# ag14774/OpenCL-Lattice-Boltzmann

Hardware: AMD Instinct MI355X
Metric: MLUPS (higher is better)
Workload: dtype f32

## Files before the change

opencl-lattice-boltzmann_amd/csrc/core_interval.h:

```cpp
#pragma once

#if defined(__HIPCC__) || defined(__CUDACC__)
#define LBM_CORE_HD __host__ __device__ inline
#else
#define LBM_CORE_HD inline
#endif

namespace lbm {

struct CoreInterval {
  int kc0, kc1;
};

LBM_CORE_HD CoreInterval core_interval(int ys, int ye, int L, int ny, bool up, bool twinned, int accel_row, int accel_row_b,
                                       bool accel_next) {
  const int n = ye - ys, d = up ? 1 : -1;
  const int lead = twinned ? 0 : L - 1, sf = twinned ? 1 : 2;
  const int r0 = up ? ys - lead : ye - 1 + lead;
  const CoreInterval none = {0, 0};
  if (n <= 0 || L < 2) return none;
  int lo = lead + L - 1, hi = n + lead - 1;
  const int k_steady = sf * (L - 1) + 1;
  if (lo < k_steady) lo = k_steady;
  if (up) {
// ... 3 lines not shown
    if (lo < kmin) lo = kmin;
  } else {
    const int kmax = (r0 - 1) - 1;
    if (hi > kmax) hi = kmax;
    const int kmin = r0 - (ny - 2) - 1;
    if (lo < kmin) lo = kmin;
  }
  if (hi - lo + 1 < 2) return none;
  const int Lacc = accel_next ? L : L - 1;
  int c0[2], c1[2], nc = 0;
  const int arows[2] = {accel_row, accel_row_b};
  for (int i = 0; i < 2; i++) {
    const int A = arows[i];
    if (A < 0 || A >= ny || Lacc <= 0) continue;
    const int kA = (A - r0) * d;
    if (kA + Lacc - 1 < lo || kA > hi) continue;
    int j = nc++;
    if (j == 1 && kA < c0[0]) { c0[1] = c0[0]; c1[1] = c1[0]; j = 0; }
    c0[j] = kA;
    c1[j] = kA + Lacc - 1;
  }
  int best0 = 0, best1 = 0;
  int start = lo;
  for (int i = 0; i <= nc; i++) {
    const int end = i < nc ? c0[i] : hi + 1;
    if (end - start > best1 - best0) { best0 = start; best1 = end; }
    if (i < nc && c1[i] + 1 > start) start = c1[i] + 1;
  }
  if (best1 - best0 < 2) return none;
  const CoreInterval r = {best0, best1};
  return r;
}

}
```

opencl-lattice-boltzmann_amd/csrc/d2q9_kernels.h:

```cpp
#pragma once
#include <type_traits>

#include <hip/hip_runtime.h>
#include <stdint.h>

#include "core_interval.h"

namespace lbm {

constexpr int kBlock = 256;

struct StepArgs {
  const float *src;
  float *dst;
  const uint8_t *mask;
  const float *south_src[3];
  const float *north_src[3];
  float *partials;
  unsigned long long plane_stride;
  unsigned long long row_stride;
  int nx, rows;
  int y_begin, y_count;
  int y_split, y_begin2;
  int accel_row;
  float omega, aw1, aw2;
};


__device__ __forceinline__ float wave_sum(float v) {
  for (int o = 32; o > 0; o >>= 1) v += __shfl_xor(v, o, 64);
  return v;
}

__device__ __forceinline__ double wave_sum(double v) {
  for (int o = 32; o > 0; o >>= 1) v += __shfl_xor(v, o, 64);
  return v;
}

typedef float v4f __attribute__((ext_vector_type(4)));
// ... 1418 lines not shown
    in.h0 = lo ? Rc[1 * ps + xhalo_w] : Rc[3 * ps + xhalo_e];
    in.h1 = lo ? Rs[5 * ps + xhalo_w] : Rs[6 * ps + xhalo_e];
    in.h2 = lo ? Rn[8 * ps + xhalo_w] : Rn[7 * ps + xhalo_e];
  }
}

typedef __attribute__((address_space(1))) v2f global_v2f;
constexpr int kPairSlotFloats = 128;
constexpr int kPairWinFloats = 9 * kPairSlotFloats;
struct PairWindow { v2f mid[3], S0[3], S1[3]; };
struct __attribute__((packed, aligned(4))) f2u { float x, y; };
__device__ __forceinline__ v2f lds_pair(const float *p) { return *reinterpret_cast<const v2f *>(p); }
__device__ __forceinline__ v2f lds_pair_shifted(const float *p) {
  const f2u t = *reinterpret_cast<const f2u *>(p);
  v2f r = {t.x, t.y};
  return r;
}
__device__ __forceinline__ void lds_pair_put(float *p, v2f v) { *reinterpret_cast<v2f *>(p) = v; }

__device__ __forceinline__ void issue_pair_loads_at(const float *Rc, size_t ps, size_t rs, int xcol, PairLoads &in) {
  unsigned xb = (unsigned)xcol * 4u;
  asm volatile("" : "+v"(xb));
  auto ld = [&](const float *p) {
    unsigned long long pk = (unsigned long long)p;
    asm volatile("" : "+s"(pk));
    return *(const global_v2f *)(pk + xb);
  };
  const float *const Rs = Rc - rs, *const Rn = Rc + rs;
  in.c[0] = ld(Rc); in.c[1] = ld(Rc + ps); in.c[3] = ld(Rc + 3 * ps);
  in.c[2] = ld(Rs + 2 * ps); in.c[5] = ld(Rs + 5 * ps); in.c[6] = ld(Rs + 6 * ps);
  in.c[4] = ld(Rn + 4 * ps); in.c[7] = ld(Rn + 7 * ps); in.c[8] = ld(Rn + 8 * ps);
}

constexpr int deep_halo_lanes(int D) { return D / 2; }
constexpr bool deep_edge_loads(int D) { return 2 * deep_halo_lanes(D) < D; }
constexpr int deep_lds_windows(int D) { return D - 1 < 4 ? D - 1 : 4; }

__device__ __forceinline__ bool strip_rows_clean(const unsigned long long *bits, int words, int strip, int lo, int hi, int ny) {
  if (bits == nullptr || hi - lo >= ny) return false;
  const unsigned long long *w = bits + (size_t)strip * words;
  unsigned long long any = 0;
  auto range = [&](int r0, int r1) {
    for (int i = r0 >> 6; i <= (r1 - 1) >> 6; i++) {
      const int b0 = r0 - 64 * i > 0 ? r0 - 64 * i : 0, b1 = r1 - 64 * i < 64 ? r1 - 64 * i : 64;
      const unsigned long long upto = b1 == 64 ? ~0ull : ((1ull << b1) - 1ull);
      any |= w[i] & upto & ~((1ull << b0) - 1ull);
    }
  };
  int l0 = lo % ny;
  if (l0 < 0) l0 += ny;
  const int l1 = l0 + (hi - lo);
  if (l1 <= ny) range(l0, l1);
  else { range(l0, ny); range(0, l1 - ny); }
  return __builtin_amdgcn_readfirstlane((int)(any == 0ull)) != 0;
}
__device__ __forceinline__ void deep_sweep_rows(bool up, bool twinned, int L, int ys, int ye, int *lo, int *hi) {
  const int lead = twinned ? 0 : L - 1, count = (ye - ys) + lead + (L - 1);
  const int first = up ? ys - lead : ye - 1 + lead - (count - 1);
  *lo = first;
  *hi = first + count;
}

static __global__ __launch_bounds__(64) void strip_row_bits(const uint8_t *mask, int nx, int rows, int strips, int lanes_out, int halo_lanes,
                                                     unsigned long long *bits, int words) {
  const int strip = blockIdx.x % strips, word = blockIdx.x / strips, lane = threadIdx.x;
  if (word >= words) return;
  const int q2 = nx >> 1;
  int qw = (strip * lanes_out + lane - halo_lanes) % q2;
  if (qw < 0) qw += q2;
  const int xcol = qw * 2;
  unsigned long long out = 0;
  for (int b = 0; b < 64; b++) {
    const int r = word * 64 + b;
    if (r >= rows) break;
    const uint32_t m = *reinterpret_cast<const uint32_t *>(mask + (size_t)r * nx + (xcol & ~3)) >> ((xcol & 2) * 8);
    if (__builtin_amdgcn_ballot_w64((m & 0xffffu) != 0) != 0ull) out |= 1ull << b;
  }
  if (lane == 0) bits[(size_t)strip * words + word] = out;
}

template <int D, int WL, bool UP, bool NT, bool OBST_PATHS, bool TWIN = false, int LT = 0, bool FREE = false>
__device__ __forceinline__ void deep_sweep(const Step2Args &a, const int L_arg, float *lds, float *partials, int pstride, int ys, int ye,
                                           int xcol, int xhalo_w, int xhalo_e, int lane, bool owner, int unit,
                                           const bool twinned_in = false, float *lds_twin = nullptr) {
  static_assert(LT >= 0 && LT <= D, "steady depth");
  const int L = LT > 0 ? LT : L_arg;
  const bool twinned = TWIN && twinned_in;
  const size_t ps = a.plane_stride;
  auto wrap = [&](int r) { return r < 0 ? r + a.ny : (r >= a.ny ? r - a.ny : r); };
  const int n = ye - ys, d = UP ? 1 : -1;
  const int lead = twinned ? 0 : L - 1;
  const int sf = twinned ? 1 : 2;
  const int r0 = UP ? ys - lead : ye - 1 + lead;
  const int last = n + lead + (L - 1) - 1;
  float sum[D];
  constexpr int NR = (D - 1 - WL) > 0 ? (D - 1 - WL) : 1;
  PairWindow w[NR];
  uint32_t m_mid[D - 1];
#pragma unroll
  for (int l = 0; l < D; l++) sum[l] = 0.f;
#pragma unroll
  for (int l = 0; l < D - 1; l++) m_mid[l] = 0;
#pragma unroll
  for (int l = 0; l < NR; l++) {
#pragma unroll
    for (int i = 0; i < 3; i++) w[l].mid[i] = w[l].S0[i] = w[l].S1[i] = splat2(0.f);
  }
  float *const lw = lds + 2 + 2 * lane;
  uint32_t accbits = 0, ownbits = 0;
  const uint32_t accmask = a.accel_next ? 0xffffffffu : ~(1u << (L - 1));
  const uint32_t mask_shift = (xcol & 2) * 8;
  PairLoads in;
  issue_pair_loads<false, deep_edge_loads(D)>(a, wrap(r0), xcol, xhalo_w, xhalo_e, lane, in);
  float *const mailbox = lw + WL * kPairWinFloats;
  auto window_read = [&](int l, int par, int k, v2f (&q)[6]) __attribute__((always_inline)) {
    if ((l - 1) < WL) {
      const float *W = lw + (l - 1) * kPairWinFloats;
// ... 21 lines not shown
#pragma unroll
      for (int kk = 0; kk < 9; kk++) {
        unsigned long long pk = (unsigned long long)(row + kk * ps);
        asm volatile("" : "+s"(pk));
        global_v2f *const q = (global_v2f *)(pk + xb);
        if (NT) __builtin_nontemporal_store(out[kk], q);
        else *q = out[kk];
      }
    }
  };
  auto store_row = [&](int kprev) __attribute__((always_inline)) { store_row_at(a.dst + (size_t)(r0 + (kprev - (L - 1)) * d) * a.row_stride); };
  constexpr bool HAS_CORE = LT > 0 && FREE && !deep_edge_loads(D);
  const float *core_src = a.src;
  float *core_dst = a.dst;
  const long long core_step = UP ? (long long)a.row_stride : -(long long)a.row_stride;
  auto iteration = [&](const int k, auto lt_tag, auto core_tag) __attribute__((always_inline)) {
    constexpr int LS = decltype(lt_tag)::value;
    constexpr bool STEADY = LS > 0;
    constexpr bool CORE = decltype(core_tag)::value;
    static_assert(!CORE || (STEADY && HAS_CORE), "the CORE form is a steady form of the free sweeps");
    const int LL = STEADY ? LS : L;
    const int par = k & 1;
    v2f top[9], pre[2][6];
    uint32_t m_top;
    if (!CORE) {
      const int row0 = wrap(r0 + k * d);
      accbits = ((accbits << 1) | ((row0 == a.accel_row || row0 == a.accel_row_b) ? 1u : 0u)) & accmask;
      ownbits = (ownbits << 1) | ((k >= lead && k <= n + lead - 1) ? 1u : 0u);
    }
    if (STEADY || k >= sf) window_read(1, par, STEADY ? -1 : k, pre[1]);
    {
      v2f g[9];
      g[0] = in.c[0]; g[2] = in.c[2]; g[4] = in.c[4];
      if (deep_edge_loads(D)) {
        g[1] = pair_from_west(in.c[1], in.h0); g[5] = pair_from_west(in.c[5], in.h1); g[8] = pair_from_west(in.c[8], in.h2);
        g[3] = pair_from_east(in.c[3], in.h0); g[6] = pair_from_east(in.c[6], in.h1); g[7] = pair_from_east(in.c[7], in.h2);
      } else {
        g[1] = pair_from_west(in.c[1]); g[5] = pair_from_west(in.c[5]); g[8] = pair_from_west(in.c[8]);
        g[3] = pair_from_east(in.c[3]); g[6] = pair_from_east(in.c[6]); g[7] = pair_from_east(in.c[7]);
      }
      m_top = FREE ? 0u : in.m >> mask_shift;
      v2f t;
      if (FREE || (OBST_PATHS && __builtin_amdgcn_ballot_w64((m_top & 0xffffu) != 0) == 0ull)) t = collide2<false>(g, m_top, a.omega, !CORE && (accbits & 1u) != 0, a.aw1, a.aw2, top);
      else t = collide2<true>(g, m_top, a.omega, (accbits & 1u) != 0, a.aw1, a.aw2, top);
      if ((CORE || (ownbits & 1u)) && owner) sum[0] += t.x + t.y;
      if (CORE) {
        store_row_at(core_dst);
        issue_pair_loads_at(core_src, ps, a.row_stride, xcol, in);
        core_dst += core_step;
        core_src += core_step;
      } else {
        if (STEADY || k - 1 >= sf * (LL - 1)) store_row(k - 1);
        issue_pair_loads<false, deep_edge_loads(D)>(a, wrap(r0 + (k < last ? k + 1 : k) * d), xcol, xhalo_w, xhalo_e, lane, in);
      }
    }
#pragma unroll
    for (int l = 1; l < D; l++) {
      if (STEADY && l >= LS) break;
      if (STEADY) __builtin_amdgcn_sched_barrier(0);
      const bool final = (l == D - 1) || (l == LL - 1);
      if (!STEADY && TWIN && (l - 1) >= WL && twinned && k == l) __syncthreads();
      v2f nxt[9];
      uint32_t m_nxt = 0;
      const bool active = STEADY || k >= sf * l;
      const bool in_lds = (l - 1) < WL;
      float *const W = lw + (l - 1) * kPairWinFloats;
      float *const Wp = W + (3 + 3 * par) * kPairSlotFloats;
      PairWindow &R = w[in_lds ? 0 : (l - 1 - WL)];
      if (active) {
        const v2f (&q)[6] = pre[l & 1];
        if (l + 1 < D && !final && (STEADY || k >= sf * (l + 1))) window_read(l + 1, par, STEADY ? -1 : k, pre[(l + 1) & 1]);
        v2f g[9];
        g[0] = q[0]; g[1] = q[1]; g[3] = q[2];
        if (UP) {
          g[2] = q[3]; g[5] = q[4]; g[6] = q[5];
          g[4] = top[4]; g[8] = pair_from_west(top[8]); g[7] = pair_from_east(top[7]);
        } else {
          g[4] = q[3]; g[8] = q[4]; g[7] = q[5];
          g[2] = top[2]; g[5] = pair_from_west(top[5]); g[6] = pair_from_east(top[6]);
        }
        m_nxt = FREE ? 0u : m_mid[l - 1];
// ... 12 lines not shown
      if (in_lds) {
        lds_pair_put(W, top[0]); lds_pair_put(W + kPairSlotFloats, top[1]); lds_pair_put(W + 2 * kPairSlotFloats, top[3]);
        lds_pair_put(Wp, UP ? top[2] : top[4]);
        lds_pair_put(Wp + kPairSlotFloats, UP ? top[5] : top[8]);
        lds_pair_put(Wp + 2 * kPairSlotFloats, UP ? top[6] : top[7]);
      } else {
        R.mid[0] = top[0]; R.mid[1] = top[1]; R.mid[2] = top[3];
#pragma unroll
        for (int i = 0; i < 3; i++) R.S0[i] = R.S1[i];
        R.S1[0] = UP ? top[2] : top[4]; R.S1[1] = UP ? top[5] : top[8]; R.S1[2] = UP ? top[6] : top[7];
      }
      if (!FREE) m_mid[l - 1] = m_top;
      if (!STEADY && TWIN && twinned && k == l - 1) {
        float *const Wt = lds_twin + 2 + 2 * lane + (in_lds ? (l - 1) * kPairWinFloats + (3 + 3 * (l & 1)) * kPairSlotFloats : WL * kPairWinFloats);
        lds_pair_put(Wt, UP ? top[4] : top[2]);
        lds_pair_put(Wt + kPairSlotFloats, UP ? top[8] : top[5]);
        lds_pair_put(Wt + 2 * kPairSlotFloats, UP ? top[7] : top[6]);
      }
      if (!active || final) break;
      if (l < D - 1) {
#pragma unroll
        for (int kk = 0; kk < 9; kk++) top[kk] = nxt[kk];
        m_top = m_nxt;
      }
    }
    if (!STEADY && TWIN && twinned && k <= L - 2) __syncthreads();
  };
  const int k_steady = sf * (L - 1) + 1;
  int k = 0;
  if (LT > 0) {
    for (; k < k_steady && k <= last; k++) iteration(k, std::integral_constant<int, 0>{}, std::false_type{});
    if constexpr (HAS_CORE) {
      CoreInterval ci = {0, 0};
      if (a.core_loop) ci = core_interval(ys, ye, L, a.ny, UP, twinned, a.accel_row, a.accel_row_b, a.accel_next != 0);
      const int kc0 = __builtin_amdgcn_readfirstlane(ci.kc0), kc1 = __builtin_amdgcn_readfirstlane(ci.kc1);
      bool core_ahead = kc1 > kc0;
      for (;;) {
        const int stop = core_ahead ? kc0 : last + 1;
        for (; k < stop; k++) iteration(k, std::integral_constant<int, LT>{}, std::false_type{});
        if (!core_ahead) break;
        core_ahead = false;
        core_src = a.src + (long long)(r0 + (kc0 + 1) * d) * (long long)a.row_stride;
        core_dst = a.dst + (long long)(r0 + (kc0 - L) * d) * (long long)a.row_stride;
        for (; k < kc1; k++) iteration(k, std::integral_constant<int, LT>{}, std::true_type{});
        ownbits = (1u << L) - 1u;
        accbits = 0;
      }
    } else {
      for (; k <= last; k++) iteration(k, std::integral_constant<int, LT>{}, std::false_type{});
    }
  } else {
    for (; k <= last; k++) iteration(k, std::integral_constant<int, 0>{}, std::false_type{});
  }
  store_row(last);
#pragma unroll
  for (int l = 0; l < D; l++) {
    if (l >= L) break;
    const float s = wave_sum(sum[l]);
    if (lane == 0) partials[(size_t)l * pstride + unit] = s;
  }
}

__device__ __forceinline__ void push_chunk_pairs(const Step2Args *la, int ys, int ye, int xcol, bool owner) {
  drain_stores();
  const HaloPeer *pp = uniform_ptr(la->peer);
  const int hi0 = __builtin_amdgcn_readfirstlane(pp->row_hi0);
  const int lo0 = __builtin_amdgcn_readfirstlane(pp->row_lo0);
  const int rows = __builtin_amdgcn_readfirstlane(pp->push_rows);
  const int buf = __builtin_amdgcn_readfirstlane(la->peer_buf) & 1;
  const int side = ys >= hi0 ? 1 : 0;
  const int base = side ? hi0 : lo0;
  if (ys < base || ye > base + rows) {
    if ((threadIdx.x & 63) == 0) atomicOr(pp->wait_err, 2u);
    return;
  }
  const size_t rs = la->row_stride, ps = la->plane_stride;
  const float *own = la->dst + xcol;
// ... 34 lines not shown
  if (slot >= us.units_per_band) return;
  const int unit0 = band * us.units_per_band + slot;
  const int sdiv = (PUSH && us.edge) ? a.strips_edge : a.strips;
  const int chunk = unit0 / sdiv;
  int strip = unit0 - chunk * sdiv;
  const int unit = unit0 + us.partial_off;
  int ys, ye;
  if (a.vmap != nullptr && !(PUSH && us.edge)) {
    const int *e = a.vtab + 2 * ((size_t)a.vmap[2 * strip + 1] * a.nchunks + chunk);
    strip = a.vmap[2 * strip];
    ys = e[0];
    ye = e[1];
  } else {
    ys = us.chunk_start[chunk];
    ye = us.chunk_start[chunk + 1];
  }
  if (ys >= ye || chunk == us.skip) {
    if (lane < nlev) partials[(size_t)lane * pstride + unit] = 0.f;
    if constexpr (PUSH) {
      const Step2Args *la = late_args<Step2Args>();
      if (us.edge && (la->peer_mode & 1)) publish_wave_when_last(la->peer, (unsigned)la->edge_units, la->seq);
    }
    return;
  }
  const int q2 = a.nx >> 1;
  const int qcol = strip * a.lanes_out + lane - HL;
  const bool owner = (lane >= HL) && (lane < HL + a.lanes_out) && (qcol < q2);
  int qw = qcol % q2;
  if (qw < 0) qw += q2;
  const int xcol = qw * 2;
  const int xhalo_w = (xcol == 0) ? a.nx - 1 : xcol - 1;
  const int xhalo_e = (xcol + 2 >= a.nx) ? 0 : xcol + 2;
  const bool up = __builtin_amdgcn_readfirstlane((int)((chunk & 1) == 0)) != 0;
  bool clean = false;
  if constexpr (LT > 0 && OBST_PATHS) {
    int lo, hi;
    deep_sweep_rows(up, false, LT, ys, ye, &lo, &hi);
    clean = strip_rows_clean(a.clean_bits, a.clean_words, strip, lo, hi, a.ny);
  }
  if (clean) {
    if constexpr (LT > 0 && OBST_PATHS) {
      if (up) deep_sweep<D, WL, true, NT, OBST_PATHS, false, LT, true>(a, nlev, lds, partials, pstride, ys, ye, xcol, xhalo_w, xhalo_e, lane, owner, unit);
      else deep_sweep<D, WL, false, NT, OBST_PATHS, false, LT, true>(a, nlev, lds, partials, pstride, ys, ye, xcol, xhalo_w, xhalo_e, lane, owner, unit);
    }
  } else if (up) {
    deep_sweep<D, WL, true, NT, OBST_PATHS, false, LT>(a, nlev, lds, partials, pstride, ys, ye, xcol, xhalo_w, xhalo_e, lane, owner, unit);
  } else {
    deep_sweep<D, WL, false, NT, OBST_PATHS, false, LT>(a, nlev, lds, partials, pstride, ys, ye, xcol, xhalo_w, xhalo_e, lane, owner, unit);
  }
  if constexpr (PUSH) {
    const Step2Args *la = late_args<Step2Args>();
    if (do_push) {
      push_chunk_pairs(la, ys, ye, xcol, owner);
      publish_wave_when_last(la->peer, (unsigned)la->edge_units, la->seq);
    }
  }
}

template <int D, bool NT, bool OBST_PATHS = false, int LT = 0, bool PUSH = false>
__global__ __launch_bounds__(128, 2) void d2q9_deep_twin(const Step2Args a, float *partials, int pstride, int nlev) {
  constexpr int WL = deep_lds_windows(D), HL = deep_halo_lanes(D);
  constexpr int kWaveFloats = WL * kPairWinFloats + (D - 1 > WL ? 3 * kPairSlotFloats : 0) + 4;
  constexpr bool EDGE_PAIRS = PUSH && D <= 5;
  __shared__ float lds[2 * kWaveFloats];
  const int lane = threadIdx.x & 63;
  const int wv = __builtin_amdgcn_readfirstlane((int)(threadIdx.x >> 6));
  const UnitSel us = select_unit<PUSH>(a, a.edge_units / 2);
  const bool do_push = PUSH && us.edge && (a.peer_mode & 1);
  if constexpr (PUSH) {
    if (us.edge && (a.peer_mode & 2)) {
      const Step2Args *la = late_args<Step2Args>();
      const HaloPeer *pp = la->peer;
      if (lane < 2) spin_on_flag(pp->wait_flags + lane, la->wait_seq, pp->wait_err, pp->wait_ticks);
    }
  }
  const int band = us.bid % us.nbands, slot = us.bid / us.nbands;
// ... 7 lines not shown
  const int unit = ((edge_wg && EDGE_PAIRS) ? 2 * pair + wv : chunk) * sdiv + strip + us.partial_off;
  int ys, ye, pys, pye;
  if (a.vmap != nullptr && !edge_wg) {
    const int *e = a.vtab + 2 * ((size_t)a.vmap[2 * strip + 1] * a.nchunks + chunk), *pe = e + (wv ? -2 : 2);
    strip = a.vmap[2 * strip];
    ys = e[0]; ye = e[1];
    pys = pe[0]; pye = pe[1];
  } else {
    ys = us.chunk_start[chunk]; ye = us.chunk_start[chunk + 1];
    pys = us.chunk_start[chunk ^ 1]; pye = us.chunk_start[(chunk ^ 1) + 1];
  }
  const bool empty = ys >= ye || (!(PUSH && us.edge) && chunk == us.skip);
  const bool twinned = !(PUSH && us.edge && !EDGE_PAIRS) && !empty && pys < pye && (chunk ^ 1) != us.skip;
  if constexpr (PUSH && !EDGE_PAIRS) {
    if (us.edge && wv == 0 && lane < nlev) partials[(size_t)lane * pstride + (a.strips_edge + strip + us.partial_off)] = 0.f;
  }
  if (empty) {
    if (lane < nlev) partials[(size_t)lane * pstride + unit] = 0.f;
    if constexpr (PUSH) {
      const Step2Args *la = late_args<Step2Args>();
      if (us.edge && (la->peer_mode & 1)) publish_wave_when_last(la->peer, (unsigned)la->edge_units, la->seq);
    }
    return;
  }
  const int q2 = a.nx >> 1;
  const int qcol = strip * a.lanes_out + lane - HL;
  const bool owner = (lane >= HL) && (lane < HL + a.lanes_out) && (qcol < q2);
  int qw = qcol % q2;
  if (qw < 0) qw += q2;
  const int xcol = qw * 2;
  const int xhalo_w = (xcol == 0) ? a.nx - 1 : xcol - 1;
  const int xhalo_e = (xcol + 2 >= a.nx) ? 0 : xcol + 2;
  float *const mine = lds + wv * kWaveFloats, *const theirs = lds + (wv ^ 1) * kWaveFloats;
  bool clean = false;
  if constexpr (LT > 0 && OBST_PATHS && D == 8) {
    int lo, hi;
    deep_sweep_rows(wv != 0, twinned, LT, ys, ye, &lo, &hi);
    clean = strip_rows_clean(a.clean_bits, a.clean_words, strip, lo, hi, a.ny);
  }
  if (clean) {
    if constexpr (LT > 0 && OBST_PATHS && D == 8) {
      if (wv != 0) deep_sweep<D, WL, true, NT, OBST_PATHS, true, LT, true>(a, nlev, mine, partials, pstride, ys, ye, xcol, xhalo_w, xhalo_e, lane, owner, unit, twinned, theirs);
      else deep_sweep<D, WL, false, NT, OBST_PATHS, true, LT, true>(a, nlev, mine, partials, pstride, ys, ye, xcol, xhalo_w, xhalo_e, lane, owner, unit, twinned, theirs);
    }
  } else if (wv != 0) {
    deep_sweep<D, WL, true, NT, OBST_PATHS, true, LT>(a, nlev, mine, partials, pstride, ys, ye, xcol, xhalo_w, xhalo_e, lane, owner, unit, twinned, theirs);
  } else {
    deep_sweep<D, WL, false, NT, OBST_PATHS, true, LT>(a, nlev, mine, partials, pstride, ys, ye, xcol, xhalo_w, xhalo_e, lane, owner, unit, twinned, theirs);
  }
  if constexpr (PUSH) {
    const Step2Args *la = late_args<Step2Args>();
    if (do_push) {
      push_chunk_pairs(la, ys, ye, xcol, owner);
      publish_wave_when_last(la->peer, (unsigned)la->edge_units, la->seq);
    }
  }
}

struct ResidentArgs {
  const float *src;
  float *dst;
  const uint8_t *mask;
  float *partials;
  unsigned long long plane_stride, row_stride, pstride;
  int nx, ny, nsteps;
  int accel_row;
  int accel_next;
  float omega, aw1, aw2;
  unsigned *words;
  float *xrows;
  unsigned seq_base;
  unsigned *err;
  unsigned long long wait_ticks;
};

__device__ __forceinline__ void resident_store(float *p, v2f v) {
// ... 453 lines not shown
```

opencl-lattice-boltzmann_amd/csrc/lbm_hip.cpp:

```cpp
#include "../../include/lbm.h"
#include "d2q9_kernels.h"
#include "deep_instances.h"
#include "chunk_schedule.h"
#include "halo_exchange.h"
#include "lbm_error.h"

#include <dlfcn.h>
#include <rccl/rccl.h>
#include <unistd.h>

#include <algorithm>
#include <cmath>
#include <cstdarg>
#include <cstdio>
#include <cstdlib>
#include <cstring>
#include <string>
#include <vector>

namespace {

thread_local std::string g_err;

int fail(int code, const char *fmt, ...) {
// ... 263 lines not shown
template <typename T>
int dev_alloc(T **p, size_t count) {
  HIP_TRY(hipMalloc(reinterpret_cast<void **>(p), count * sizeof(T)));
  return LBM_OK;
}

int step_blocks(const lbm_ctx *c, int work_rows) {
  const int vec = c->vec4 ? 4 : 1;
  const long threads = (long)(c->p.nx / vec) * work_rows;
  int nb = div_up(threads, kBlock);
  if (c->grid_blocks > 0) nb = std::min(nb, c->grid_blocks);
  return std::max(1, nb);
}

bool windows_in_lds(const lbm_ctx *c) { return c->windows < 0 ? kStep3LdsDefault : c->windows != 0; }
int step3_load_bufs(const lbm_ctx *c) { return c->load_bufs > 0 ? c->load_bufs : (windows_in_lds(c) ? 1 : 2); }

bool step3_can_pair(const lbm_ctx *c) { return windows_in_lds(c) && step3_load_bufs(c) == 1 && c->pair != 0; }

int step3_sched_waves(const lbm_ctx *c) {
  if (c->sched_waves > 0) return c->sched_waves;
  if (!windows_in_lds(c)) return 1;
  if (step3_can_pair(c)) return 2;
  return (long)c->p.nx * c->rows_min <= 800L * 1024 ? 1 : 2;
}
int step4_sched_waves(const lbm_ctx *c) { return c->sched_waves > 0 ? c->sched_waves : 2; }

int pair_taper(const lbm_ctx *c) { return c->pair_taper >= 0 ? c->pair_taper : kPairTaper32; }

bool fuse_possible(const lbm_ctx *c) {
  if (!c->vec4 || c->p.nx < 256) return false;
  return c->rows_min >= 8;
}
bool deep_possible(const lbm_ctx *c) {
  return fuse_possible(c) && c->rows_min >= 4 * kDeepSteps && (!c->halo_mode || c->halo_depth >= kDeepMin);
}
constexpr long kTwinDeepCells = 3L << 20;
constexpr long kSlabDeepCells = 3L << 20;
constexpr long kSlabTwinCells = 300L * 1024;
constexpr int kOneRoundRows = 160;
constexpr int kMaxHeavyStrips = 4;
bool compact_transport(const lbm_ctx *c) { return c->halo_mode && c->transport_eff == TRANSPORT_PEER && c->compact != 0; }
bool stageable_transport(const lbm_ctx *c) {
  if (!c->halo_mode || c->transport_eff != TRANSPORT_RCCL || c->compact == 0 || c->slabs.empty()) return false;
  for (const Slab &s : c->slabs)
    if (!s.can_wait_value) return false;
  return true;
}
bool slab_twin5(const lbm_ctx *c) {
  if ((long)c->p.nx * c->rows_min <= kSlabTwinCells || (long)c->p.nx * c->rows_min >= kSlabDeepCells) return false;
  const bool transport_ok = compact_transport(c) || (stageable_transport(c) && c->halo_depth == kDeepTwinDefault);
  return transport_ok && (c->halo_depth == kDeepTwinDefault || c->halo_depth == kMultiMaxT) && fuse_possible(c) && c->rows_min >= 4 * kDeepTwinDefault &&
         c->pair != 0 && c->multistep <= 0 && (c->fuse < 0 || c->fuse == kDeepTwinDefault) && c->twin_steps <= 0;
}
int twin_cap(const lbm_ctx *c) {
  if (slab_twin5(c)) return kDeepTwinDefault;
  if (c->twin_steps > 0) return c->twin_steps;
  return (long)c->p.nx * c->rows_min >= kTwinDeepCells ? kDeepTwinSteps : kDeepTwinDefault;
}
bool deep_twin_effective(const lbm_ctx *c) {
  if (c->halo_mode || c->slabs.empty() || !c->slabs[0].f6_twin.paired) return false;
  return c->pair != 0;
}
int fuse_level(const lbm_ctx *c) {
  if (!fuse_possible(c)) return 0;
  if (slab_twin5(c)) return kDeepTwinDefault;
  int lvl;
  if (c->fuse >= 0) {
    lvl = c->fuse == 0 ? 0 : (c->fuse >= 3 ? c->fuse : 2);
  } else {
    const long cells = (long)c->p.nx * c->rows_min;
    lvl = cells >= 1280L * 1024 ? 4 : (cells > 450L * 1024 ? 3 : 2);
    if (deep_possible(c) && (cells >= kSlabDeepCells || (cells > 300L * 1024 && deep_twin_effective(c)))) lvl = kDeepSteps;
  }
  if (lvl > 4 && !(lvl >= kDeepMin && lvl <= kDeepSteps && deep_possible(c))) lvl = 4;
  if (lvl >= kDeepMin && c->halo_mode) lvl = std::min(lvl, c->halo_depth);
  if (lvl == 4 && ((c->halo_mode && c->halo_depth < 4) || !windows_in_lds(c))) lvl = 3;
  if (lvl == 3 && c->halo_mode && c->halo_depth < 3) lvl = 2;
  return lvl;
}

bool resident_effective(const lbm_ctx *c) {
  if (c->halo_mode || c->slabs.size() != 1 || c->slabs[0].res_bands <= 0) return false;
  if (c->resident >= 0) return c->resident > 0;
  return c->fuse < 0 && c->multistep < 0 && (long)c->p.nx * c->p.ny >= 200L * 1024;
}
const void *resident_kernel(int bh) {
  return bh == 2 ? (const void *)d2q9_resident<2> : bh == 4 ? (const void *)d2q9_resident<4> : (const void *)d2q9_resident<6>;
}
int resident_geometry(const lbm_ctx *c, Slab &s) {
  s.res_bh = s.res_w = s.res_bands = 0;
  if (c->halo_mode || c->resident == 0 || c->p.nx % 4 != 0 || c->p.nx < 128 || c->p.nx > 1024) return LBM_OK;
  const int W = div_up(c->p.nx, 128);
  if (set_dev(s)) return LBM_ERR_HIP;
  int bh = 0;
  for (int cand : {2, 4, 6}) {
    if (c->p.ny % cand != 0) continue;
    int per_cu = 0;
// ... 384 lines not shown
      for (int y = 0; y < s.edge_rows; y += ec) tab.push_back(s.row0 + s.rows - s.edge_rows + y);
      tab.push_back(s.row0 + s.rows);
      if (tab.size() % 2 == 0) tab.push_back(s.row0 + s.rows);
      if (set_dev(s)) return LBM_ERR_HIP;
      if (e.chunk_start) HIP_TRY(hipFree(e.chunk_start));
      e.chunk_start = nullptr;
      if (dev_alloc(&e.chunk_start, tab.size())) return LBM_ERR_HIP;
      HIP_TRY(hipMemcpy(e.chunk_start, tab.data(), tab.size() * sizeof(int), hipMemcpyHostToDevice));
      e.nchunks = (int)tab.size() - 1;
      e.skip = n_edge_chunks;
      e.nbands = 1;
      e.units_per_band = e.nchunks * s.strips;
      e.units = e.units_per_band;
      const int i0 = s.row0 + s.edge_rows, i1 = s.row0 + s.rows - s.edge_rows;
      if (i1 > i0) {
        const int rsv = compact_sets(c) ? 4 * n_edge_chunks * s.strips : 2 * n_edge_chunks * s.strips;
        if (int rc = fuse_schedule(s, i0, i1, cmax, cmin, true, s.f_main, 2, rsv)) return rc;
        if (int rc = fuse_schedule_pairs(c, s, i0, i1, c3max, c3min, s.f3_main, step3_sched_waves(c), rsv, step3_can_pair(c))) return rc;
        if (int rc = fuse_schedule_pairs(c, s, i0, i1, c4max, c4min, s.f4_main, step4_sched_waves(c), rsv, windows_in_lds(c))) return rc;
      } else {
        s.f_main.units = s.f3_main.units = s.f4_main.units = 0;
        s.f_main.paired = s.f3_main.paired = s.f4_main.paired = false;
      }
      s.nb_total = std::max(s.nb_total, std::max(s.f_main.units, std::max(s.f3_main.units, s.f4_main.units)) + e.units);
    } else {
      if (int rc = fuse_schedule(s, 0, s.rows, cmax, cmin, true, s.f_main)) return rc;
      s.nb_total = std::max(s.nb_total, s.f_main.units);
      if (int rc = fuse_schedule_pairs(c, s, 0, s.rows, c3max, c3min, s.f3_main, step3_sched_waves(c), 0, step3_can_pair(c))) return rc;
      s.nb_total = std::max(s.nb_total, s.f3_main.units);
      if (int rc = fuse_schedule_pairs(c, s, 0, s.rows, c4max, c4min, s.f4_main, step4_sched_waves(c), 0, windows_in_lds(c))) return rc;
      s.nb_total = std::max(s.nb_total, s.f4_main.units);
    }
    if (int rc = deep_geometry(c, s)) return rc;
  }
  if (int rc = resident_geometry(c, s)) return rc;
  return LBM_OK;
}

bool nt_effective(const lbm_ctx *c) {
  if (c->nt_stores >= 0) return c->nt_stores != 0;
  const size_t grid_bytes = c->slabs[0].row_stride * c->slabs[0].ext_rows * sizeof(float);
  return 2 * grid_bytes > ((size_t)192 << 20);
}

int effective_mode(const lbm_ctx *c) {
  if (!c->vec4) return LM_SCALAR;
  const bool wave_rows = (c->p.nx % 256 == 0);
  int m = c->variant > 0 ? c->variant - 1 : (wave_rows ? LM_DPP : LM_SCALAR);
  if ((m == LM_DPP || m == LM_LDS) && !wave_rows) m = LM_SCALAR;
  return m;
}

enum { KIND_NONE = 0, KIND_SINGLE = 1, KIND_FUSED2 = 2, KIND_MULTI = 3, KIND_FUSED3 = 4, KIND_FUSED4 = 5, KIND_DEEP = 6, KIND_RESIDENT = 7 };
enum { FORM_ONE_SLAB = 0, FORM_TWO_STREAM = 1, FORM_COMPACT = 2, FORM_STAGED = 3 };

struct LaunchPlan {
  int kind = KIND_SINGLE;
  int cap = 1;
  int window_kind = KIND_SINGLE;
  int fuse_lvl = 0;
  int form = FORM_ONE_SLAB;
  bool multi = false;
  bool pairs = false;
  bool twin = false;
  bool twin5 = false;
  bool nt = false, paths = true, steady = true;
// ... 1574 lines not shown
    if (e != hipSuccess) return fail(LBM_ERR_HIP, "HIP error in reynolds: %s", hipGetErrorString(e));
  }
  const float viscosity = 1.0f / 6.0f * (2.0f / c->p.omega - 1.0f);
  const float av = (float)(tot * (double)c->p.free_cells_inv);
  *reynolds_out = av * c->p.reynolds_dim / viscosity;
  return LBM_OK;
}

int lbm_set_option(lbm_ctx *c, const char *key, long value) {
  if (!c || !key) return fail(LBM_ERR_ARG, "NULL argument");
  if (!strcmp(key, "variant")) {
    if (value < 0 || value > 4) return fail(LBM_ERR_ARG, "variant must be 0..4");
    c->variant = (int)value;
    return LBM_OK;
  }
  if (!strcmp(key, "grid_blocks")) {
    if (value < 0) return fail(LBM_ERR_ARG, "grid_blocks must be >= 0");
    if (int rc = sync_all(c)) return rc;
    c->grid_blocks = (int)value;
    return rebuild_geometry(c);
  }
  if (!strcmp(key, "nt_stores")) {
    if (value < -1 || value > 1) return fail(LBM_ERR_ARG, "nt_stores must be -1 (auto), 0 or 1");
    c->nt_stores = (int)value;
    return LBM_OK;
  }
  if (!strcmp(key, "nt_loads")) {
    if (value < -1 || value > 2) return fail(LBM_ERR_ARG, "nt_loads must be -1 (auto), 0, 1 or 2");
    c->nt_loads = (int)value;
    return c->halo_mode ? rebuild_geometry(c) : LBM_OK;
  }
  if (!strcmp(key, "fuse")) {
    if (value < -1 || value > kDeepSteps) return fail(LBM_ERR_ARG, "fuse must be -1 (auto), 0, 1 (or 2), 3 .. 8");
    c->fuse = (int)value;
    return c->halo_mode ? rebuild_geometry(c) : LBM_OK;
  }
  if (!strcmp(key, "twin_steps")) {
    if (value != 0 && (value < 2 || value > kDeepTwinSteps)) return fail(LBM_ERR_ARG, "twin_steps must be 0 (auto) or 2..%d", kDeepTwinSteps);
    if (int rc = sync_all(c)) return rc;
    c->twin_steps = (int)value;
    return rebuild_geometry(c);
  }
  if (!strcmp(key, "edge_aware")) {
    if (value < -1 || value > 1) return fail(LBM_ERR_ARG, "edge_aware must be -1 (auto), 0 or 1");
    if (int rc = sync_all(c)) return rc;
    c->edge_aware = (int)value;
    return rebuild_geometry(c);
  }
  if (!strcmp(key, "steady")) {
    if (value < -1 || value > 1) return fail(LBM_ERR_ARG, "steady must be -1 (auto), 0 or 1");
    c->steady = (int)value;
    return LBM_OK;
  }
  if (!strcmp(key, "obst_paths")) {
    if (value < -1 || value > 1) return fail(LBM_ERR_ARG, "obst_paths must be -1 (auto), 0 or 1");
    c->obst_paths = (int)value;
    return LBM_OK;
  }
  if (!strcmp(key, "balance")) {
    if (value < -1 || value > 1) return fail(LBM_ERR_ARG, "balance must be -1 (auto), 0 or 1");
    if (int rc = sync_all(c)) return rc;
    c->balance = (int)value;
    return rebuild_geometry(c);
  }
  if (!strcmp(key, "free_sweeps")) {
    if (value < -1 || value > 1) return fail(LBM_ERR_ARG, "free_sweeps must be -1 (auto), 0 or 1");
    c->free_sweeps = (int)value;
    return LBM_OK;
  }
  if (!strcmp(key, "core_loop")) {
    if (value < -1 || value > 1) return fail(LBM_ERR_ARG, "core_loop must be -1 (auto), 0 or 1");
    c->core_loop = (int)value;
    return LBM_OK;
  }
  if (!strcmp(key, "tile_shape")) {
    if (value < -1 || value > 2) return fail(LBM_ERR_ARG, "tile_shape must be -1..2");
    if (int rc = sync_all(c)) return rc;
    c->tile_shape = (int)value;
    return rebuild_geometry(c);
  }
  if (!strcmp(key, "pair")) {
    if (int rc = sync_all(c)) return rc;
    c->pair = (int)value;
    return rebuild_geometry(c);
  }
  if (!strcmp(key, "windows") || !strcmp(key, "load_bufs") || !strcmp(key, "sched_waves")) {
    if (value < -1 || value > 2) return fail(LBM_ERR_ARG, "%s out of range", key);
    if (key[0] == 'w' && value == 0) return fail(LBM_ERR_ARG, "windows 0 (register windows of d2q9_step3) was removed: -1 or 1");
    if (key[0] == 'l' && value == 2) return fail(LBM_ERR_ARG, "load_bufs 2 (two row-sets of loads in flight in d2q9_step3) was removed: 0 or 1");
    if (int rc = sync_all(c)) return rc;
    (key[0] == 'w' ? c->windows : (key[0] == 'l' ? c->load_bufs : c->sched_waves)) = (int)value;
    return rebuild_geometry(c);
  }
  if (!strcmp(key, "transport")) {
    if (!c->halo_mode) return fail(LBM_ERR_STATE, "a context without halo rows has no transport");
    if (int rc = sync_all(c)) return rc;
    if (value == TRANSPORT_RCCL) {
      for (const Slab &s : c->slabs)
        if (!s.comm) return fail(LBM_ERR_STATE, "no RCCL communicator: create the context with a comm_id (or default transport 1)");
    } else if (value == TRANSPORT_PEER) {
      for (const Slab &s : c->slabs)
        if (!s.south.connected || !s.north.connected) return fail(LBM_ERR_STATE, "peers are not connected (lbm_connect_peers)");
    } else {
      return fail(LBM_ERR_ARG, "transport must be 1 (RCCL send/recv) or 3 (peer stores)");
    }
    c->transport_eff = (int)value;
    return rebuild_geometry(c);
// ... 78 lines not shown
    c->pair_taper = (int)value;
    return rebuild_geometry(c);
  }
  return fail(LBM_ERR_ARG, "unknown option '%s'", key);
}

int lbm_get_option(const lbm_ctx *c, const char *key, long *value) {
  if (!c || !key || !value) return fail(LBM_ERR_ARG, "NULL argument");
  const LaunchPlan p = resolve_plan(c);
  const Slab *s0 = c->slabs.empty() ? nullptr : &c->slabs[0];
  if (!strcmp(key, "variant")) *value = effective_mode(c) + 1;
  else if (!strcmp(key, "grid_blocks")) *value = s0 ? s0->nb_main : 0;
  else if (!strcmp(key, "nt_stores")) *value = nt_effective(c);
  else if (!strcmp(key, "fuse")) *value = p.fuse_lvl >= 3 ? p.fuse_lvl : (p.fuse_lvl ? 1 : 0);
  else if (!strcmp(key, "multistep")) *value = p.kind == KIND_MULTI ? p.cap : 0;
  else if (!strcmp(key, "resident")) *value = p.kind == KIND_RESIDENT ? s0->res_bh : 0;
  else if (!strcmp(key, "chunk_rows")) *value = c->chunk_rows;
  else if (!strcmp(key, "pair_taper")) *value = pair_taper(c);
  else if (!strcmp(key, "windows")) *value = windows_in_lds(c);
  else if (!strcmp(key, "pair")) *value = p.pairs;
  else if (!strcmp(key, "load_bufs")) *value = step3_load_bufs(c);
  else if (!strcmp(key, "launch_steps")) *value = p.cap;
  else if (!strcmp(key, "fuse_units"))
    *value = !s0 ? 0 : (p.twin ? s0->f6_main.units : set_geom(p, *s0, p.window_kind).main->units) + set_geom(p, *s0, p.window_kind).edge->units;
  else if (!strcmp(key, "transport")) *value = c->transport_eff;
  else if (!strcmp(key, "steady")) *value = c->steady != 0;
  else if (!strcmp(key, "balance")) {
    const int vstrips = s0 && p.fuse_lvl >= kDeepMin ? set_geom(p, *s0, KIND_DEEP).main->vstrips : 0;
    *value = vstrips > 0 ? vstrips - s0->strips2 : 0;
  }
  else if (!strcmp(key, "free_sweeps"))
    *value = s0 && p.fuse_lvl >= kDeepMin && clean_bits_for(c, *s0, *set_geom(p, *s0, KIND_DEEP).main) != nullptr;
  else if (!strcmp(key, "core_loop")) *value = c->core_loop != 0;
  else if (!strcmp(key, "halo_sync")) *value = c->halo_sync;
  else if (!strcmp(key, "halo_timeout_ms")) *value = (long)c->halo_timeout_ms;
  else if (!strcmp(key, "push_release")) *value = c->slabs.empty() ? 0 : push_release_effective(c, c->slabs[0]);
  else if (!strcmp(key, "debug_stale_exchange")) *value = c->stale_exchange;
  else if (!strcmp(key, "compact")) *value = p.compact();
  else if (!strcmp(key, "halo_depth")) *value = c->halo_mode ? c->halo_depth : 0;
  else if (!strcmp(key, "nslabs")) *value = c->nslabs_global;
  else if (!strcmp(key, "cus")) *value = s0 ? s0->cus : 0;
  else return fail(LBM_ERR_ARG, "unknown option '%s'", key);
  return LBM_OK;
}

int lbm_valu_rate(int launches, double *tera_lane_instr_per_s) {
  if (!tera_lane_instr_per_s || launches < 1) return fail(LBM_ERR_ARG, "bad argument");
  const int nb = 256 * 8, iters = 4096;
  float *out = nullptr;
  HIP_TRY(hipMalloc((void **)&out, (size_t)nb * kBlock * sizeof(float)));
  hipEvent_t t0, t1;
  hipEventCreate(&t0);
  hipEventCreate(&t1);
  hipLaunchKernelGGL(lbm::valu_spin, dim3(nb), dim3(kBlock), 0, 0, out, iters, 0.5f);
  hipEventRecord(t0, 0);
  for (int i = 0; i < launches; i++) hipLaunchKernelGGL(lbm::valu_spin, dim3(nb), dim3(kBlock), 0, 0, out, iters, 0.5f);
  hipEventRecord(t1, 0);
  const hipError_t e = hipEventSynchronize(t1);
  float ms = 0.f;
  hipEventElapsedTime(&ms, t0, t1);
  hipEventDestroy(t0);
  hipEventDestroy(t1);
  hipFree(out);
  if (e != hipSuccess || ms <= 0.f) return fail(LBM_ERR_HIP, "valu_spin: %s", hipGetErrorString(e));
  *tera_lane_instr_per_s = (double)nb * kBlock * (double)iters * 32.0 * launches / (ms * 1e-3) / 1e12;
  return LBM_OK;
// ... 72 lines not shown
```

Before: 480,200.

## Load shifted west/east populations directly in core loop; enable deep fusion for narrow grids

In the steady core loop, the six diagonal and horizontal populations are now read with unaligned pair loads offset by one float, so each lane gets its neighbour values straight from memory. This replaces cross-lane shuffles through pair_from_west/east. The shifted form is used only for strips whose columns are away from the periodic x edges. On entry and exit of the core loop the in-flight loads are converted or reissued to keep the two forms consistent. Separately, deep temporal fusion is now allowed for grids 128-255 wide when fuse is set explicitly, and a read-only core_shift option is added. The trade is 4-byte-aligned vector loads that may split cache lines, in exchange for fewer lane-permute instructions.

```diff
diff --git a/opencl-lattice-boltzmann_amd/csrc/core_interval.h b/opencl-lattice-boltzmann_amd/csrc/core_interval.h
--- a/opencl-lattice-boltzmann_amd/csrc/core_interval.h
+++ b/opencl-lattice-boltzmann_amd/csrc/core_interval.h
@@ -59,4 +59,9 @@
   return r;
 }
 
+LBM_CORE_HD bool core_shift_columns(int strip, int lanes_out, int halo_lanes, int nx) {
+  const int q0 = strip * lanes_out - halo_lanes;
+  return q0 >= 1 && q0 + 63 <= nx / 2 - 2;
 }
+
+}
diff --git a/opencl-lattice-boltzmann_amd/csrc/d2q9_kernels.h b/opencl-lattice-boltzmann_amd/csrc/d2q9_kernels.h
--- a/opencl-lattice-boltzmann_amd/csrc/d2q9_kernels.h
+++ b/opencl-lattice-boltzmann_amd/csrc/d2q9_kernels.h
@@ -5,6 +5,11 @@
 #include <stdint.h>
 
 #include "core_interval.h"
+
+#ifndef LBM_CORE_SHIFT
+#define LBM_CORE_SHIFT 1
+#endif
+static_assert(LBM_CORE_SHIFT >= 0 && LBM_CORE_SHIFT <= 1, "LBM_CORE_SHIFT is 0 or 1");
 
 namespace lbm {
 
@@ -1489,6 +1494,30 @@
   in.c[4] = ld(Rn + 4 * ps); in.c[7] = ld(Rn + 7 * ps); in.c[8] = ld(Rn + 8 * ps);
 }
 
+typedef float v2f_a4 __attribute__((ext_vector_type(2), aligned(4)));
+typedef __attribute__((address_space(1))) v2f_a4 global_v2f_a4;
+typedef __attribute__((address_space(1))) char global_char;
+__device__ __forceinline__ void issue_pair_loads_shifted_at(const float *Rc, size_t ps, size_t rs, int xcol, PairLoads &in) {
+  unsigned xb = (unsigned)xcol * 4u;
+  asm volatile("" : "+v"(xb));
+  auto ld = [&](const float *p) {
+    unsigned long long pk = (unsigned long long)p;
+    asm volatile("" : "+s"(pk));
+    return *(const global_v2f *)(pk + xb);
+  };
+  auto ld_shifted = [&](const float *p, int shift) {
+    unsigned long long pk = (unsigned long long)p;
+    asm volatile("" : "+s"(pk));
+    const global_char *const q = (const global_char *)(pk + xb) + shift;
+    const v2f r = *(const global_v2f_a4 *)q;
+    return r;
+  };
+  const float *const Rs = Rc - rs, *const Rn = Rc + rs;
+  in.c[0] = ld(Rc); in.c[1] = ld_shifted(Rc + ps, -4); in.c[3] = ld_shifted(Rc + 3 * ps, 4);
+  in.c[2] = ld(Rs + 2 * ps); in.c[5] = ld_shifted(Rs + 5 * ps, -4); in.c[6] = ld_shifted(Rs + 6 * ps, 4);
+  in.c[4] = ld(Rn + 4 * ps); in.c[7] = ld_shifted(Rn + 7 * ps, 4); in.c[8] = ld_shifted(Rn + 8 * ps, -4);
+}
+
 constexpr int deep_halo_lanes(int D) { return D / 2; }
 constexpr bool deep_edge_loads(int D) { return 2 * deep_halo_lanes(D) < D; }
 constexpr int deep_lds_windows(int D) { return D - 1 < 4 ? D - 1 : 4; }
@@ -1539,7 +1568,7 @@
 template <int D, int WL, bool UP, bool NT, bool OBST_PATHS, bool TWIN = false, int LT = 0, bool FREE = false>
 __device__ __forceinline__ void deep_sweep(const Step2Args &a, const int L_arg, float *lds, float *partials, int pstride, int ys, int ye,
                                            int xcol, int xhalo_w, int xhalo_e, int lane, bool owner, int unit,
-                                           const bool twinned_in = false, float *lds_twin = nullptr) {
+                                           const bool twinned_in = false, float *lds_twin = nullptr, const bool shift_cols = false) {
   static_assert(LT >= 0 && LT <= D, "steady depth");
   const int L = LT > 0 ? LT : L_arg;
   const bool twinned = TWIN && twinned_in;
@@ -1627,7 +1656,10 @@
     {
       v2f g[9];
       g[0] = in.c[0]; g[2] = in.c[2]; g[4] = in.c[4];
-      if (deep_edge_loads(D)) {
+      if (CORE && LBM_CORE_SHIFT >= 1) {
+        g[1] = in.c[1]; g[5] = in.c[5]; g[8] = in.c[8];
+        g[3] = in.c[3]; g[6] = in.c[6]; g[7] = in.c[7];
+      } else if (deep_edge_loads(D)) {
         g[1] = pair_from_west(in.c[1], in.h0); g[5] = pair_from_west(in.c[5], in.h1); g[8] = pair_from_west(in.c[8], in.h2);
         g[3] = pair_from_east(in.c[3], in.h0); g[6] = pair_from_east(in.c[6], in.h1); g[7] = pair_from_east(in.c[7], in.h2);
       } else {
@@ -1641,7 +1673,8 @@
       if ((CORE || (ownbits & 1u)) && owner) sum[0] += t.x + t.y;
       if (CORE) {
         store_row_at(core_dst);
-        issue_pair_loads_at(core_src, ps, a.row_stride, xcol, in);
+        if (LBM_CORE_SHIFT >= 1) issue_pair_loads_shifted_at(core_src, ps, a.row_stride, xcol, in);
+        else issue_pair_loads_at(core_src, ps, a.row_stride, xcol, in);
         core_dst += core_step;
         core_src += core_step;
       } else {
@@ -1720,7 +1753,7 @@
     for (; k < k_steady && k <= last; k++) iteration(k, std::integral_constant<int, 0>{}, std::false_type{});
     if constexpr (HAS_CORE) {
       CoreInterval ci = {0, 0};
-      if (a.core_loop) ci = core_interval(ys, ye, L, a.ny, UP, twinned, a.accel_row, a.accel_row_b, a.accel_next != 0);
+      if (a.core_loop && (LBM_CORE_SHIFT == 0 || shift_cols)) ci = core_interval(ys, ye, L, a.ny, UP, twinned, a.accel_row, a.accel_row_b, a.accel_next != 0);
       const int kc0 = __builtin_amdgcn_readfirstlane(ci.kc0), kc1 = __builtin_amdgcn_readfirstlane(ci.kc1);
       bool core_ahead = kc1 > kc0;
       for (;;) {
@@ -1730,7 +1763,12 @@
         core_ahead = false;
         core_src = a.src + (long long)(r0 + (kc0 + 1) * d) * (long long)a.row_stride;
         core_dst = a.dst + (long long)(r0 + (kc0 - L) * d) * (long long)a.row_stride;
+        if (LBM_CORE_SHIFT >= 1) {
+          in.c[1] = pair_from_west(in.c[1]); in.c[5] = pair_from_west(in.c[5]); in.c[8] = pair_from_west(in.c[8]);
+          in.c[3] = pair_from_east(in.c[3]); in.c[6] = pair_from_east(in.c[6]); in.c[7] = pair_from_east(in.c[7]);
+        }
         for (; k < kc1; k++) iteration(k, std::integral_constant<int, LT>{}, std::true_type{});
+        if (LBM_CORE_SHIFT >= 1) issue_pair_loads_at(core_src - core_step, ps, a.row_stride, xcol, in);
         ownbits = (1u << L) - 1u;
         accbits = 0;
       }
@@ -1831,6 +1869,7 @@
   const int xhalo_w = (xcol == 0) ? a.nx - 1 : xcol - 1;
   const int xhalo_e = (xcol + 2 >= a.nx) ? 0 : xcol + 2;
   const bool up = __builtin_amdgcn_readfirstlane((int)((chunk & 1) == 0)) != 0;
+  const bool shift_cols = __builtin_amdgcn_readfirstlane((int)core_shift_columns(strip, a.lanes_out, HL, a.nx)) != 0;
   bool clean = false;
   if constexpr (LT > 0 && OBST_PATHS) {
     int lo, hi;
@@ -1839,8 +1878,8 @@
   }
   if (clean) {
     if constexpr (LT > 0 && OBST_PATHS) {
-      if (up) deep_sweep<D, WL, true, NT, OBST_PATHS, false, LT, true>(a, nlev, lds, partials, pstride, ys, ye, xcol, xhalo_w, xhalo_e, lane, owner, unit);
-      else deep_sweep<D, WL, false, NT, OBST_PATHS, false, LT, true>(a, nlev, lds, partials, pstride, ys, ye, xcol, xhalo_w, xhalo_e, lane, owner, unit);
+      if (up) deep_sweep<D, WL, true, NT, OBST_PATHS, false, LT, true>(a, nlev, lds, partials, pstride, ys, ye, xcol, xhalo_w, xhalo_e, lane, owner, unit, false, nullptr, shift_cols);
+      else deep_sweep<D, WL, false, NT, OBST_PATHS, false, LT, true>(a, nlev, lds, partials, pstride, ys, ye, xcol, xhalo_w, xhalo_e, lane, owner, unit, false, nullptr, shift_cols);
     }
   } else if (up) {
     deep_sweep<D, WL, true, NT, OBST_PATHS, false, LT>(a, nlev, lds, partials, pstride, ys, ye, xcol, xhalo_w, xhalo_e, lane, owner, unit);
@@ -1914,6 +1953,7 @@
   const int xhalo_w = (xcol == 0) ? a.nx - 1 : xcol - 1;
   const int xhalo_e = (xcol + 2 >= a.nx) ? 0 : xcol + 2;
   float *const mine = lds + wv * kWaveFloats, *const theirs = lds + (wv ^ 1) * kWaveFloats;
+  const bool shift_cols = __builtin_amdgcn_readfirstlane((int)core_shift_columns(strip, a.lanes_out, HL, a.nx)) != 0;
   bool clean = false;
   if constexpr (LT > 0 && OBST_PATHS && D == 8) {
     int lo, hi;
@@ -1922,8 +1962,8 @@
   }
   if (clean) {
     if constexpr (LT > 0 && OBST_PATHS && D == 8) {
-      if (wv != 0) deep_sweep<D, WL, true, NT, OBST_PATHS, true, LT, true>(a, nlev, mine, partials, pstride, ys, ye, xcol, xhalo_w, xhalo_e, lane, owner, unit, twinned, theirs);
-      else deep_sweep<D, WL, false, NT, OBST_PATHS, true, LT, true>(a, nlev, mine, partials, pstride, ys, ye, xcol, xhalo_w, xhalo_e, lane, owner, unit, twinned, theirs);
+      if (wv != 0) deep_sweep<D, WL, true, NT, OBST_PATHS, true, LT, true>(a, nlev, mine, partials, pstride, ys, ye, xcol, xhalo_w, xhalo_e, lane, owner, unit, twinned, theirs, shift_cols);
+      else deep_sweep<D, WL, false, NT, OBST_PATHS, true, LT, true>(a, nlev, mine, partials, pstride, ys, ye, xcol, xhalo_w, xhalo_e, lane, owner, unit, twinned, theirs, shift_cols);
     }
   } else if (wv != 0) {
     deep_sweep<D, WL, true, NT, OBST_PATHS, true, LT>(a, nlev, mine, partials, pstride, ys, ye, xcol, xhalo_w, xhalo_e, lane, owner, unit, twinned, theirs);
diff --git a/opencl-lattice-boltzmann_amd/csrc/lbm_hip.cpp b/opencl-lattice-boltzmann_amd/csrc/lbm_hip.cpp
--- a/opencl-lattice-boltzmann_amd/csrc/lbm_hip.cpp
+++ b/opencl-lattice-boltzmann_amd/csrc/lbm_hip.cpp
@@ -319,8 +319,11 @@
   if (!c->vec4 || c->p.nx < 256) return false;
   return c->rows_min >= 8;
 }
+bool deep_narrow(const lbm_ctx *c) {
+  return c->vec4 && c->p.nx >= 128 && c->p.nx < 256 && !c->halo_mode && c->fuse >= kDeepMin && c->fuse <= kDeepSteps;
+}
 bool deep_possible(const lbm_ctx *c) {
-  return fuse_possible(c) && c->rows_min >= 4 * kDeepSteps && (!c->halo_mode || c->halo_depth >= kDeepMin);
+  return (fuse_possible(c) || deep_narrow(c)) && c->rows_min >= 4 * kDeepSteps && (!c->halo_mode || c->halo_depth >= kDeepMin);
 }
 constexpr long kTwinDeepCells = 3L << 20;
 constexpr long kSlabDeepCells = 3L << 20;
@@ -350,7 +353,7 @@
   return c->pair != 0;
 }
 int fuse_level(const lbm_ctx *c) {
-  if (!fuse_possible(c)) return 0;
+  if (!fuse_possible(c)) return deep_narrow(c) && deep_possible(c) ? c->fuse : 0;
   if (slab_twin5(c)) return kDeepTwinDefault;
   int lvl;
   if (c->fuse >= 0) {
@@ -801,6 +804,8 @@
       s.nb_total = std::max(s.nb_total, s.f4_main.units);
     }
     if (int rc = deep_geometry(c, s)) return rc;
+  } else if (deep_narrow(c)) {
+    if (int rc = deep_geometry(c, s)) return rc;
   }
   if (int rc = resident_geometry(c, s)) return rc;
   return LBM_OK;
@@ -2441,6 +2446,11 @@
   }
   if (!strcmp(key, "fuse")) {
     if (value < -1 || value > kDeepSteps) return fail(LBM_ERR_ARG, "fuse must be -1 (auto), 0, 1 (or 2), 3 .. 8");
+    if (!c->halo_mode && c->p.nx < 256) {
+      if (int rc = sync_all(c)) return rc;
+      c->fuse = (int)value;
+      return rebuild_geometry(c);
+    }
     c->fuse = (int)value;
     return c->halo_mode ? rebuild_geometry(c) : LBM_OK;
   }
@@ -2482,6 +2492,8 @@
     c->core_loop = (int)value;
     return LBM_OK;
   }
+  if (!strcmp(key, "core_shift"))
+    return fail(LBM_ERR_ARG, "core_shift is read-only: the library was built with LBM_CORE_SHIFT=%d", (int)LBM_CORE_SHIFT);
   if (!strcmp(key, "tile_shape")) {
     if (value < -1 || value > 2) return fail(LBM_ERR_ARG, "tile_shape must be -1..2");
     if (int rc = sync_all(c)) return rc;
@@ -2626,6 +2638,7 @@
   else if (!strcmp(key, "free_sweeps"))
     *value = s0 && p.fuse_lvl >= kDeepMin && clean_bits_for(c, *s0, *set_geom(p, *s0, KIND_DEEP).main) != nullptr;
   else if (!strcmp(key, "core_loop")) *value = c->core_loop != 0;
+  else if (!strcmp(key, "core_shift")) *value = LBM_CORE_SHIFT;
   else if (!strcmp(key, "halo_sync")) *value = c->halo_sync;
   else if (!strcmp(key, "halo_timeout_ms")) *value = (long)c->halo_timeout_ms;
   else if (!strcmp(key, "push_release")) *value = c->slabs.empty() ? 0 : push_release_effective(c, c->slabs[0]);
```

Measured after the change: 480,900, median of 2. Within noise of the previous version (+0.2%).
